# RHnejad/3D_PoseEstimation

Measured on AMD Instinct MI355X. Metric: poses/sec fwd+bwd, 17-joint lifting batch 4096; MPJPE vs ref, higher is better.
Workload: dtype f16x3 (two fp16 planes per fp32 operand, 3 fp16 MFMAs per product, fp32 accumulate); 1 GPU; BASELINE configs[1]: phase1_lifting LinearModel 34-1024-2x(1024-1024)-51, BN+ReLU+Dropout(0.5), one train_1.py step = zero_grad+forward+MSE+backward+AdamW; launch=eager (one call per kernel), per_gpu_batch=4096, global_batch=4096, parallelism=dp1

## Files before the change

3d_poseestimation_amd/_lib.py:

```python
import ctypes
import os

import torch

_HERE = os.path.dirname(os.path.abspath(__file__))
LIB_PATH = os.environ.get("POSELIFT_LIB") or os.path.join(_HERE, "csrc", "libposelift.so")

PL_F32, PL_BF16, PL_BF16X6, PL_F16X3 = 0, 1, 2, 3


GATHER_FN = ctypes.CFUNCTYPE(ctypes.c_int, ctypes.c_void_p, ctypes.c_void_p, ctypes.c_int64, ctypes.c_void_p)


class PLSync(ctypes.Structure):
    _fields_ = [("world", ctypes.c_int32), ("rank", ctypes.c_int32), ("gather", GATHER_FN),
                ("user", ctypes.c_void_p)]


class PLL1Term(ctypes.Structure):
    _fields_ = [("a", ctypes.c_void_p), ("b", ctypes.c_void_p), ("n", ctypes.c_int64),
                ("da", ctypes.c_void_p), ("db", ctypes.c_void_p)]


L1_MAX_TERMS = 8
# ... 84 lines not shown
_D = ctypes.POINTER(PLDesc)
SIGNATURES = {
    "pl_version": (_c.c_int, []),
    "pl_last_error": (_c.c_char_p, []),
    "pl_num_hidden": (_c.c_int64, [_D]),
    "pl_param_tensors": (_c.c_int64, [_D]),
    "pl_param_offset": (_c.c_int64, [_D, _c.c_int64]),
    "pl_param_numel": (_c.c_int64, [_D, _c.c_int64]),
    "pl_param_arena_floats": (_c.c_int64, [_D]),
    "pl_workspace_bytes": (_c.c_size_t, [_D, _c.c_int64]),
    "pl_workspace_view": (_c.c_int, [_D, _c.c_int64, _c.c_int, _c.c_int64,
                                     _c.POINTER(_c.c_size_t), _c.POINTER(_c.c_size_t)]),
    "pl_workspace_bitmap_format": (_c.c_int, [_D, _c.c_int64, _c.c_int64]),
    "pl_lifter_fwd_eval": (_c.c_int, [_D, _P, _P, _c.c_int64, _P, _c.c_size_t, _P]),
    "pl_lifter_fwd_train": (_c.c_int, [_D, _P, _P, _c.c_int64, _P, _c.c_size_t, _c.c_uint64,
                                       _c.c_uint64, _P, _P]),
    "pl_lifter_bwd": (_c.c_int, [_D, _P, _P, _c.c_int64, _P, _c.c_size_t, _P, _P, _P]),
    "pl_lifter_fwd_eval_saved": (_c.c_int, [_D, _P, _P, _c.c_int64, _P, _c.c_size_t, _P]),
    "pl_lifter_bwd_eval": (_c.c_int, [_D, _P, _P, _c.c_int64, _P, _c.c_size_t, _P, _P, _P]),
    "pl_lifter_bwd_layers": (_c.c_int, [_D, _P, _P, _c.c_int64, _P, _c.c_size_t, _P, _P, _c.c_int, _c.c_int, _P]),
    "pl_lifter_train_fwd_bwd": (_c.c_int, [_D, _P, _P, _c.c_int64, _P, _c.c_size_t, _c.c_uint64, _c.c_uint64,
                                           _P, _P, _P, _c.c_int, _c.c_int, _P]),
    "pl_lifter_step_carries_adamw": (_c.c_int, [_D, _c.c_int64]),
    "pl_lifter_train_step": (_c.c_int, [_D, _P, _P, _c.c_int64, _P, _c.c_size_t, _c.c_uint64, _c.c_uint64,
                                        _P, _P, _P, _c.POINTER(PLAdamWStep), _P]),
    "pl_lifter_train_fwd_bwd_crit": (_c.c_int, [_D, _P, _P, _c.c_int64, _P, _c.c_size_t, _c.c_uint64, _c.c_uint64,
                                                _c.POINTER(PLCriterion), _P, _P, _P, _c.c_int, _c.c_int, _P]),
    "pl_lifter_train_step_crit": (_c.c_int, [_D, _P, _P, _c.c_int64, _P, _c.c_size_t, _c.c_uint64, _c.c_uint64,
                                             _c.POINTER(PLCriterion), _P, _P, _P, _c.POINTER(PLAdamWStep), _P]),
    "pl_pose_loss_scratch_bytes": (_c.c_size_t, [_c.c_int64, _c.c_int64, _c.POINTER(PLCriterion)]),
    "pl_pose_loss_fwd_bwd": (_c.c_int, [_P, _P, _c.c_int64, _c.c_int64, _c.POINTER(PLCriterion), _c.c_float, _P, _P, _P, _P]),
    "pl_mse_scratch_bytes": (_c.c_size_t, [_c.c_int64]),
    "pl_mse_fwd_bwd": (_c.c_int, [_P, _P, _c.c_int64, _c.c_float, _P, _P, _P, _P]),
    "pl_l1_scratch_bytes": (_c.c_size_t, [_c.c_int]),
    "pl_l1_terms_fwd_bwd": (_c.c_int, [_c.POINTER(PLL1Term), _c.c_int, _c.c_float, _P, _P, _P]),
    "pl_mpjpe_scratch_bytes": (_c.c_size_t, [_c.c_int64, _c.c_int64]),
    "pl_mpjpe_accum": (_c.c_int, [_P, _P, _c.c_int64, _c.c_int64, _P, _P, _P]),
    "pl_pose_errors": (_c.c_int, [_P, _P, _c.c_int64, _c.c_int64, _P, _P, _P]),
    "pl_pose_errors_host": (_c.c_int, [_P, _P, _c.c_int64, _c.c_int64, _P, _P]),
    "pl_pose_errors_t": (_c.c_int, [_P, _P, _c.c_int64, _c.c_int64, _P, _P, _P, _P, _P]),
    "pl_mpjpe_accum_t": (_c.c_int, [_P, _P, _c.c_int64, _c.c_int64, _P, _P, _P, _P, _P]),
    "pl_pose_metrics_scratch_bytes": (_c.c_size_t, [_c.c_int64, _c.c_int64, _c.c_int, _c.c_int]),
    "pl_pose_metrics_accum": (_c.c_int, [_P, _c.c_int64, _c.c_int64, _P, _c.c_int, _P, _c.c_int, _P, _P, _P, _P, _P]),
    "pl_adamw_flat": (_c.c_int, [_P, _P, _P, _P, _c.c_int64, _c.c_float, _c.c_float, _c.c_float,
                                 _c.c_float, _c.c_float, _c.c_int64, _c.c_float, _P]),
    "pl_adamw_flat_dev": (_c.c_int, [_P, _P, _P, _P, _c.c_int64, _P, _c.c_float, _c.c_float, _c.c_float,
# ... 247 lines not shown
```

3d_poseestimation_amd/csrc/api.hip:

```cpp
#include <stdarg.h>
#include <stdio.h>
#include <stdlib.h>

#include <vector>

#include "adamw.h"
#include "pl_internal.h"

namespace pl {

static thread_local char g_err[512] = "";

void set_error(const char* fmt, ...) {
  va_list ap;
  va_start(ap, fmt);
  vsnprintf(g_err, sizeof(g_err), fmt, ap);
  va_end(ap);
}

namespace {

inline int64_t align_up(int64_t v, int64_t a) { return (v + a - 1) / a * a; }

int check_desc(const PLDesc* d, bool need_arenas) {
// ... 651 lines not shown
namespace pl {
namespace {

struct BwdCtx {
  const PLDesc* d;
  const Ws& w;
  const ParamLayout& P;
  void* ws;
  hipStream_t s;
  const float *x, *dy;
  float *dx, *grads;
  int B, H, O;
  int l_hi, l_lo;
  float kscale;
  bool eval_bn;
  bool small, sl;
  bool top_fused;
  float* loss_out;
  int n_loss_part;
  float loss_inv_n;
  const PLAdamWStep* adam;
  bool adam_rides;
  std::vector<RowJob> jobs;

  float* buf(size_t off) const { return f32(ws, off); }
  float* GA() const { return buf(w.ga); }
  float* GB() const { return buf(w.gb); }
  float* DZ() const { return buf(w.dz); }
  int64_t BH() const { return (int64_t)B * H; }
  const float* gin(int l) const { return (l % 2 == 1) ? GB() : GA(); }
  float* dzbuf(int l) const { return (sl && (l & 1)) ? GB() : DZ(); }
  bool planes_pair(int l) const { return w.layer[l].bwd == Bwd::PlanesPair; }
  float* dzs(int l) const { return (planes_pair(l) && w.pkind == 2) ? buf(w.dzscale) + 2 * l : nullptr; }
  void job(const float* part, float* out, int R, int Hj, int kind, int transK) { jobs.push_back(RowJob{part, out, R, Hj, kind, transK}); }
  SmallBnLayer bn_layer(int l) const {
    const Layer y = layer_of(d, P, grads, l);
    return SmallBnLayer{saved_of(w, ws, l), y.bn.gamma, y.ggamma, y.gbeta, y.gb};
  }
  AdamWRide ride(int64_t lo, int64_t hi) const {
    AdamWRide r = {};
    r.p = const_cast<float*>(d->params) + lo; r.g = grads + lo; r.m = adam->m + lo; r.v = adam->v + lo; r.n = hi - lo;
    r.lr = adam->lr; r.beta1 = adam->beta1; r.beta2 = adam->beta2; r.eps = adam->eps; r.wd = adam->weight_decay; r.gscale = 1.0f;
    r.t = adam->t; r.lr_dev = adam->lr_dev; r.t_dev = adam->t_dev;
    return r;
  }
};

int bnr_amax_pairs(const BwdCtx& c, int l) { return (c.B / 64) * (c.H / (l == c.w.L - 1 ? 32 : 64)); }
BnrEpilogue bnr_of(const BwdCtx& c, int l) {
  const BnSaved sv = saved_of(c.w, c.ws, l);
  const bool scaled = c.w.pkind == 2 && l > 0;
  const BnrSlab slab = bnr_slab(c.d, c.w, c.ws, c.B / 64, scaled ? bnr_amax_pairs(c, l) : 0, c.eval_bn);
  BnrEpilogue b = {};
  b.z = sv.z; b.bits = sv.bits; b.mean = sv.mean; b.rstd = sv.rstd; b.kscale = c.kscale;
  b.part_dy = slab.mine; b.part_dyz = slab.mine + (size_t)(c.B / 64) * c.H;
  b.amax = scaled ? slab.amax_mine : nullptr;
  return b;
}
void set_bnr(GemmArgs& e, const BnrEpilogue& b) {
  e.bnr_z = b.z; e.bnr_bits = b.bits; e.bnr_mean = b.mean; e.bnr_rstd = b.rstd; e.bnr_kscale = b.kscale;
  e.bnr_part_dy = b.part_dy; e.bnr_part_dyz = b.part_dyz; e.bnr_amax = b.amax;
}

int bwd_output(BwdCtx& c) {
  const Ws& w = c.w;
  const int Bi = c.B, H = c.H, O = c.O;
  const float* W2 = c.d->params + c.P.off[4 * w.L];
  float* gW2 = c.grads + c.P.off[4 * w.L];
  float* gb2 = c.grads + c.P.off[4 * w.L + 1];
  const float* h = c.buf(w.act[w.L - 1]);
  if (c.top_fused) {
    SmallTopBwdArgs a = {};
    a.dy = c.dy; a.W2 = W2; a.h = h; a.B = Bi; a.H = H; a.O = O; a.gout = c.GA(); a.dW2 = gW2; a.db2 = gb2;
    a.top = c.bn_layer(w.L - 1); a.kscale = c.kscale; a.dz_top = c.DZ();
    a.mpart = c.buf(w.mse); a.np = c.n_loss_part; a.inv_n = c.loss_inv_n; a.loss = c.loss_out;
    a.tick = const_cast<uint64_t*>(c.d->step_dev);
    return launch_small_top_bwd(a, c.s);
  }
  if (w.out_skinny) {
    SkinnyWideInArgs wi = {};
    wi.X = c.dy; wi.D = h; wi.B = Bi; wi.K = O; wi.H = H; wi.part = c.buf(w.skp_out); wi.xsum = c.buf(w.outpart);
    PL_TRY(launch_skinny_wide_in(wi, c.s));
    c.job(c.buf(w.skp_out), gW2, skinny_in_chunks(Bi), O * H, 0, 0);
    c.job(c.buf(w.outpart), gb2, skinny_in_chunks(Bi), O, 0, 0);
// ... 53 lines not shown
  a.dz = c.planes_pair(l) ? nullptr : c.DZ(); a.part_db = c.buf(w.dbpart[l]);
  a.planes.scale = 1.0f; a.planes.dyn = dzs;
  if (c.planes_pair(l)) { a.planes.h = u16(c.ws, w.dzp); a.planes.l = a.planes.h + c.BH(); a.planes.kind = w.pkind; }
  PL_TRY(launch_bn_bwd_dz(a, c.s));
  c.job(c.buf(w.dbpart[l]), ly.gb, w.RC, H, 0, 0);
  return PL_OK;
}

int bwd_layer_linear(BwdCtx& c, int l) {
  const Ws& w = c.w;
  const PLDesc* d = c.d;
  const int Bi = c.B, H = c.H;
  hipStream_t s = c.s;
  const Layer ly = layer_of(d, c.P, c.grads, l);
  const LayerRoute& r = w.layer[l];
  float* const GA = c.GA();
  float* const GB = c.GB();
  float* const DZ = c.DZ();
  float* const DZl = c.dzbuf(l);
  float* slabs = c.buf(w.slabs);
  const float* a_in = l == 0 ? c.x : (w.planes ? nullptr : c.buf(w.act[l - 1]));
  if (c.planes_pair(l)) {
    float* dzs = c.dzs(l);
    const int64_t BH = c.BH();
    const int splits = tn_splits(H, H, Bi);
    PlanesGemmArgs nn = planes_args(w.pkind, u16(c.ws, w.dzp), BH, H, wplane(d, w, c.ws, l), (int64_t)H * H, H,
                                    (l % 2 == 1) ? GA : GB, Bi, H, H, 1.0f / kWeightPlaneScale, dzs ? dzs + 1 : nullptr);
    if (l % 2 == 1) nn.e.addend = GA;
    if (!c.eval_bn && w.layer[l - 1].bnr_fused) set_bnr(nn.e, bnr_of(c, l - 1));
    float* wsl = c.buf(w.wslab[l]);
    PlanesGemmArgs tn = planes_args(w.pkind, u16(c.ws, w.dzp), BH, H, u16(c.ws, w.actp[l - 1]), BH, H,
                                    splits > 1 ? wsl : ly.gW, H, H, Bi, 1.0f / kActPlaneScale, dzs ? dzs + 1 : nullptr);
    tn.e.split_k = splits;
    PL_TRY(launch_gemm_planes_pair(nn, tn, s));
    if (splits > 1) c.job(wsl, ly.gW, splits, H * H, 1, 0);
  } else if (l > 0) {
    GemmArgs g = {};
    g.A = DZl; g.B = ly.W; g.M = Bi; g.N = H; g.K = H; g.lda = H; g.ldb = H; g.ldc = H; g.split_k = 1;
    if (l % 2 == 1) { g.C = GA; g.addend = GA; } else { g.C = GB; }
    g.arith = arith_of(d);
    g.thin_scratch = slabs; g.thin_scratch_floats = w.slab_floats;
    GemmArgs t = {};
    t.arith = g.arith;
    t.A = DZl; t.B = a_in; t.M = H; t.N = H; t.K = Bi; t.lda = H; t.ldb = H; t.ldc = H; t.split_k = 1; t.C = ly.gW;
    if (c.sl && (r.bwd == Bwd::SmallLayer || r.bwd == Bwd::SmallLayerDw)) {
      const bool dw_rides = r.bwd == Bwd::SmallLayerDw;
      if (l - 1 < c.l_lo) {
        PL_TRY(launch_gemm_f32(kNN, g, s));
        return launch_gemm_f32(kTN, t, s);
      }
      const bool w1 = l == 1 && w.layer[0].bwd == Bwd::InAbove;
      AdamWRide ar = {};
      if (c.adam_rides) ar = c.ride(c.P.off[4 * l + 1], l == w.L - 1 ? c.P.total : c.P.off[4 * (l + 1) + 1]);
      SmallLayerBwdArgs a = {};
      a.dz = DZl; a.W = ly.W; a.B = Bi; a.H = H; a.K = H;
      if (l % 2 == 1) { a.addend = GA; a.gout = GA; }
      a.below = c.bn_layer(l - 1); a.kscale = c.kscale; a.dz_lo = c.dzbuf(l - 1);
      if (dw_rides) { a.a_in = a_in; a.dW = ly.gW; }
// ... 33 lines not shown
                    float* loss_out = nullptr, int n_loss_part = 0, float loss_inv_n = 0.f, const PLAdamWStep* adam = nullptr) {
  PL_TRY(check_desc(d, true));
  if (!x || !dy || !grads) PL_FAIL(PL_EINVAL, "pl_lifter_bwd: null x/dy/flat_grads");
  if (B <= 0) PL_FAIL(PL_ESHAPE, "pl_lifter_bwd: B=%lld", (long long)B);
  const Ws w = plan(d, B);
  PL_TRY(check_ws(w, ws, ws_bytes));
  const ParamLayout P = param_layout(d);
  BwdCtx c = {d, w, P, ws, (hipStream_t)stream, x, dy, dx, grads, (int)B, d->hidden, d->out_dim, l_hi, l_lo};
  c.kscale = eval_bn ? 1.0f : dropout_key(d->p_dropout, 0, 0, 0, nullptr, nullptr).kscale;
  c.eval_bn = eval_bn;
  c.small = !eval_bn && w.bn_small;
  c.sl = !eval_bn && w.small_layer;
  c.top_fused = do_output && !eval_bn && w.top_fused && l_hi == w.L - 1 && l_hi >= l_lo;
  c.loss_out = loss_out;
  c.n_loss_part = n_loss_part;
  c.loss_inv_n = loss_inv_n;
  c.adam = adam;
  c.adam_rides = adam && c.top_fused && l_lo == 0 && w.adam_rides;
  if (do_output) PL_TRY(bwd_output(c));
  for (int l = l_hi; l >= l_lo; --l) {
    PL_TRY(bwd_layer_bn(c, l));
    PL_TRY(bwd_layer_linear(c, l));
  }
  float inv_n = 0.f;
  uint64_t* tick = nullptr;
  if (loss_out && !c.top_fused) {
    c.job(f32(ws, w.mse), loss_out, c.n_loss_part, 1, 2, 0);
    inv_n = loss_inv_n;
    tick = const_cast<uint64_t*>(d->step_dev);
  }
  if (!c.jobs.empty()) PL_TRY(launch_reduce_rows_multi(c.jobs.data(), (int)c.jobs.size(), inv_n, tick, c.s));
  if (adam) {
    const int64_t n = c.adam_rides ? (w.L > 1 ? P.off[4 * 1 + 1] : P.total) : P.total;
    const AdamWArgs a = {const_cast<float*>(d->params), grads, adam->m, adam->v, n,
                         {adam->lr, adam->beta1, adam->beta2, adam->eps, adam->weight_decay, 1.0f, adam->t, adam->lr_dev,
                          adam->t_dev}};
    PL_TRY(launch_adamw(a, c.s));
  }
  return PL_OK;
}

extern "C" int pl_lifter_bwd(const PLDesc* d, const float* x, const float* dy, int64_t B, void* ws,
                             size_t ws_bytes, float* dx, float* grads, void* stream) {
  if (!d) PL_FAIL(PL_EINVAL, "descriptor is NULL");
  return bwd_impl(d, x, dy, B, ws, ws_bytes, dx, grads, stream, true, 2 * d->num_stage, 0);
}
// ... 272 lines not shown
                            double* flops_total) {
  if (!ms_total || !launches || !flops_total) PL_FAIL(PL_EINVAL, "pl_prof_read: null pointer");
  return prof_read(min_flops, max_flops, ms_total, launches, flops_total);
}

static int train_fwd_bwd_impl(const PLDesc* d, const float* x, const float* target, int64_t B, void* ws, size_t ws_bytes,
                              uint64_t seed, uint64_t step, const PLCriterion* crit, float* y, float* loss, float* grads, int hi,
                              int lo, void* stream, const PLAdamWStep* adam);

extern "C" int pl_lifter_train_fwd_bwd_crit(const PLDesc* d, const float* x, const float* target, int64_t B, void* ws,
                                            size_t ws_bytes, uint64_t seed, uint64_t step, const PLCriterion* crit, float* y,
                                            float* loss, float* grads, int hi, int lo, void* stream) {
  return train_fwd_bwd_impl(d, x, target, B, ws, ws_bytes, seed, step, crit, y, loss, grads, hi, lo, stream, nullptr);
}
extern "C" int pl_lifter_train_fwd_bwd(const PLDesc* d, const float* x, const float* target, int64_t B, void* ws,
                                       size_t ws_bytes, uint64_t seed, uint64_t step, float* y, float* loss,
                                       float* grads, int hi, int lo, void* stream) {
  return pl_lifter_train_fwd_bwd_crit(d, x, target, B, ws, ws_bytes, seed, step, nullptr, y, loss, grads, hi, lo, stream);
}

extern "C" int pl_lifter_step_carries_adamw(const PLDesc* d, int64_t B) {
  PL_TRY(check_desc(d, false));
  return B > 0 && plan(d, B).adam_rides ? 1 : 0;
}

extern "C" int pl_lifter_train_step_crit(const PLDesc* d, const float* x, const float* target, int64_t B, void* ws,
                                         size_t ws_bytes, uint64_t seed, uint64_t step, const PLCriterion* crit, float* y,
                                         float* loss, float* grads, const PLAdamWStep* opt, void* stream) {
  if (!opt || !opt->m || !opt->v || (opt->lr_dev != nullptr) != (opt->t_dev != nullptr) || opt->t < (opt->t_dev ? 0 : 1))
    PL_FAIL(PL_EINVAL, "pl_lifter_train_step: bad optimizer description");
  if (!d) PL_FAIL(PL_EINVAL, "descriptor is NULL");
  return train_fwd_bwd_impl(d, x, target, B, ws, ws_bytes, seed, step, crit, y, loss, grads, 1 + 2 * d->num_stage, 0, stream, opt);
}
extern "C" int pl_lifter_train_step(const PLDesc* d, const float* x, const float* target, int64_t B, void* ws, size_t ws_bytes,
                                    uint64_t seed, uint64_t step, float* y, float* loss, float* grads, const PLAdamWStep* opt,
                                    void* stream) {
  return pl_lifter_train_step_crit(d, x, target, B, ws, ws_bytes, seed, step, nullptr, y, loss, grads, opt, stream);
}

static int train_fwd_bwd_impl(const PLDesc* d, const float* x, const float* target, int64_t B, void* ws, size_t ws_bytes,
                              uint64_t seed, uint64_t step, const PLCriterion* crit, float* y, float* loss, float* grads, int hi,
                              int lo, void* stream, const PLAdamWStep* adam) {
  PL_TRY(check_desc(d, true));
  if (!x || !target || !y || !loss || !grads) PL_FAIL(PL_EINVAL, "pl_lifter_train_fwd_bwd: null pointer");
  if (B <= 0) PL_FAIL(PL_ESHAPE, "pl_lifter_train_fwd_bwd: B=%lld", (long long)B);
  PL_TRY(check_range(d, hi, lo, "pl_lifter_train_fwd_bwd"));
// ... 28 lines not shown
```

3d_poseestimation_amd/csrc/gemm_planes.h:

```cpp
#pragma once
#include <hip/hip_runtime.h>
#include <stddef.h>
#include <stdint.h>

#include <type_traits>

namespace plp {

typedef __bf16 bf16x8 __attribute__((ext_vector_type(8)));
typedef _Float16 f16x8 __attribute__((ext_vector_type(8)));
typedef short s16x4 __attribute__((ext_vector_type(4)));
typedef short s16x8 __attribute__((ext_vector_type(8)));

enum PlanesMode { kBf16 = 0, kBf16x6 = 1, kF16x3 = 2 };
template <int MODE> struct ModeCfg;
template <> struct ModeCfg<kBf16>   { static constexpr int NPL = 1, NACC = 1, NPROD = 1; };
template <> struct ModeCfg<kBf16x6> { static constexpr int NPL = 3, NACC = 1, NPROD = 6; };
template <> struct ModeCfg<kF16x3>  { static constexpr int NPL = 2, NACC = 2, NPROD = 3; };
constexpr float kF16LoScale = 2048.0f;

struct PlanesArgs {
  const __bf16* A;
  const __bf16* B;
  float* C;
  int M, N, K;
  int lda, ldb, ldc;
  int split_k;
  size_t a_plane, b_plane;
  int cv_cin, cv_h, cv_w, cv_ho, cv_wo, cv_kw, cv_stride, cv_stride_w, cv_pad_h, cv_pad_w;
};

template <int BKX, int NPL, int NST = 3>
struct PlanesCfg {
  static constexpr int OPP = 128 * BKX * 2;
  static constexpr int STAGE = 2 * NPL * OPP;
  static constexpr int LDS = NST * STAGE;
  static constexpr int NJ = BKX / 16;
  static constexpr int NDMA = 2 * NPL * NJ;
};

#define PLP_BLDS16(rsrc, lp, voff, soff) \
  __builtin_amdgcn_raw_ptr_buffer_load_lds((rsrc), (__attribute__((address_space(3))) void*)(lp), 16, (voff), (soff), 0, 0)

template <int N>
__device__ __forceinline__ void wait_vmcnt() {
  asm volatile("s_waitcnt vmcnt(%0)" ::"n"(N) : "memory");
}

template <int NDS, int NVM, int NMF>
__device__ __forceinline__ void sched_half() {
  constexpr int QV0 = (NDS + 1) / 2;
#pragma unroll
// ... 11 lines not shown
```

3d_poseestimation_amd/csrc/gemm_planes.hip:

```cpp
#include "gemm_planes16.h"
#include "pl_internal.h"
#include "plane_store.h"

namespace pl {
namespace {

struct PlanesKern {
  plp::PlanesArgs p;
  GemmArgs e;
  float out_scale;
  const float* dyn_inv;
  int nt_store;
};

__device__ __forceinline__ float xadd16(const float v) {
  const auto r = __builtin_amdgcn_permlane16_swap(__float_as_uint(v), __float_as_uint(v), false, false);
  return __uint_as_float(r[0]) + __uint_as_float(r[1]);
}
__device__ __forceinline__ float xadd32(const float v) {
  const auto r = __builtin_amdgcn_permlane32_swap(__float_as_uint(v), __float_as_uint(v), false, false);
  return __uint_as_float(r[0]) + __uint_as_float(r[1]);
}
__device__ __forceinline__ float4 xadd_rows(float4 s) {
  s.x = xadd32(xadd16(s.x)); s.y = xadd32(xadd16(s.y)); s.z = xadd32(xadd16(s.z)); s.w = xadd32(xadd16(s.w));
// ... 381 lines not shown
  __device__ __forceinline__ void finish() {
    if constexpr (BNR) {
      const GemmArgs& e = k.e;
      const int N = e.N;
      s1 = xadd_rows(s1);
      s2 = xadd_rows(s2);
      if ((lane >> 4) == 0) {
        *reinterpret_cast<float4*>(e.bnr_part_dy + (size_t)rg * N + col0) = s1;
        *reinterpret_cast<float4*>(e.bnr_part_dyz + (size_t)rg * N + col0) = s2;
      }
      if (e.bnr_amax) {
#pragma unroll
        for (int o = 32; o > 0; o >>= 1) { mxd = fmaxf(mxd, __shfl_xor(mxd, o)); mxz = fmaxf(mxz, __shfl_xor(mxz, o)); }
        if (lane == 0) {
          float* q = e.bnr_amax + ((size_t)rg * (N >> 6) + cb) * 2;
          q[0] = mxd; q[1] = mxz;
        }
      }
    }
  }
};

template <int MODE, bool HAND, bool ADD = false, bool BNR = false>
__global__ __launch_bounds__(512) void planes_gemm_chain_kernel(PlanesKern k0, PlanesKern k1) {
  constexpr int BEHIND = HAND ? plp::kHandBytes : stage_bytes<32>();
  static_assert(ring_bytes<MODE>() + BEHIND <= 160 * 1024 && stage_bytes<32>() <= plp::kHandBytes, "LDS per CU");
  __shared__ __attribute__((aligned(16))) char lds[ring_bytes<MODE>() + BEHIND];
  const int lane = threadIdx.x & 63, wave = threadIdx.x >> 6;
  const int wm = (wave & 3) >> 1, wn = wave & 1;
  float* ldsw = reinterpret_cast<float*>(lds + ring_bytes<MODE>()) + (wave & 3) * 32 * 68;
  auto epi0 = [&](plp::f32x4v (&acc)[plp::ModeCfg<MODE>::NACC][4][4], const int m0, const int n0, const int slice) {
    if constexpr (!HAND) acc_epilogue<MODE, 32, false>(k0, acc, ldsw, m0, n0, slice, wm, wn, lane);
  };
  auto epi1 = [&](plp::f32x4v (&acc)[plp::ModeCfg<MODE>::NACC][4][4], const int m0, const int n0, const int slice) {
    acc_epilogue<MODE, 32, false>(k1, acc, ldsw, m0, n0, slice, wm, wn, lane);
  };
  if constexpr (HAND) {
    ChainHand<MODE, ADD, BNR> hand(k0, reinterpret_cast<float*>(lds + ring_bytes<MODE>()) + (wave & 3) * 64 * 64, lane);
    plp::planes_run16_chain<MODE>(k0.p, k1.p, blockIdx.x, gridDim.x, lds, hand, epi0, epi1);
  } else {
    NoHand hand;
    plp::planes_run16_chain<MODE>(k0.p, k1.p, blockIdx.x, gridDim.x, lds, hand, epi0, epi1);
  }
}

template <int MODE>
__global__ __launch_bounds__(512) void planes_gemm_dual_kernel(PlanesKern k0, PlanesKern k1, int n0) {
  __shared__ __attribute__((aligned(16))) char lds[lds_bytes<MODE>()];
  const int b = blockIdx.x;
  if (b < n0)
    planes_body<false, true, MODE>(k0, b, n0, n0, lds);
  else
    planes_body<true, true, MODE>(k1, b - n0, gridDim.x - n0, gridDim.x - n0, lds);
}

PlanesKern kern_of(const PlanesGemmArgs& a) {
  PlanesKern k = {};
  k.p.A = reinterpret_cast<const __bf16*>(a.A);
  k.p.B = reinterpret_cast<const __bf16*>(a.B);
  k.p.C = a.e.C;
  k.p.M = a.e.M; k.p.N = a.e.N; k.p.K = a.e.K;
  k.p.lda = a.lda; k.p.ldb = a.ldb; k.p.ldc = a.e.ldc;
  k.p.split_k = a.e.split_k;
  k.p.a_plane = (size_t)a.a_plane; k.p.b_plane = (size_t)a.b_plane;
  k.e = a.e;
// ... 68 lines not shown
    }
    if (r.edge) launch(Bool<true>{}, Int<0>{}); else launch(Bool<false>{}, Int<0>{});
  };
  switch (layout) {
    case kNT: one_item(Bool<false>{}, Bool<false>{}, Int<1>{}); break;
    case kNN: one_item(Bool<false>{}, Bool<true>{}, Int<0>{}); break;
    case kTN: one_item(Bool<true>{}, Bool<true>{}, Int<2>{}); break;
    default: PL_FAIL(PL_EINVAL, "gemm_planes: bad layout %d", (int)layout);
  }
  return PL_OK;
}

enum class PairRoute { Chain, ChainHand, Dual };
bool chain_hand_ok(const GemmArgs& e) {
  return e.C && splits_of(e) == 1 && !e.bias && !e.col_scale && !e.relu && !e.resid && !e.cpl_kind && !e.stat_sum && !e.scat_on;
}
PairRoute pair_route(const PlanesGemmArgs& nn, const PlanesGemmArgs& tn) {
  const int ts = splits_of(tn.e);
  const bool chain = grid_of(nn) == grid_of(tn) && nn.e.K % 32 == 0 && nn.e.K >= 64 && tn.e.K % (32 * ts) == 0 && tn.e.K >= 32 * ts;
  if (!chain) return PairRoute::Dual;
  const int nk1 = tn.e.K / (32 * ts);
  return nk1 >= plp::kChainMinNk1 && chain_hand_ok(nn.e) ? PairRoute::ChainHand : PairRoute::Chain;
}
template <int MODE>
void launch_pair(PairRoute r, const PlanesKern& k0, const PlanesKern& k1, int g0, int g1, hipStream_t s) {
  const dim3 block(512);
  if (r == PairRoute::ChainHand) {
    auto launch = [&](auto ADD, auto BNR) {
      hipLaunchKernelGGL((planes_gemm_chain_kernel<MODE, true, decltype(ADD)::value, decltype(BNR)::value>), dim3(g0), block, 0, s, k0, k1);
    };
    auto with_bnr = [&](auto ADD) { if (k0.e.bnr_z) launch(ADD, Bool<true>{}); else launch(ADD, Bool<false>{}); };
    if (k0.e.addend) with_bnr(Bool<true>{}); else with_bnr(Bool<false>{});
  } else if (r == PairRoute::Chain) {
    hipLaunchKernelGGL((planes_gemm_chain_kernel<MODE, false>), dim3(g0), block, 0, s, k0, k1);
  } else {
    hipLaunchKernelGGL((planes_gemm_dual_kernel<MODE>), dim3(g0 + g1), block, 0, s, k0, k1, g0);
  }
}

}

bool planes_gemm_ok(GemmLayout layout, const PlanesGemmArgs& a) {
  const GemmArgs& e = a.e;
  const int splits = splits_of(e);
  if (a.mode != plp::kBf16 && a.mode != plp::kF16x3) return false;
  if (!a.A || !a.B || (!e.C && !e.cpl_kind) || e.M <= 0 || e.N <= 0 || e.K <= 0) return false;
  if (e.cpl_kind && (splits > 1 || !e.cpl_h || (e.cpl_kind == 2 && !e.cpl_l) ||
                     ((reinterpret_cast<uintptr_t>(e.cpl_h) | reinterpret_cast<uintptr_t>(e.cpl_l)) & 7)))
    return false;
  if (e.K % (32 * splits)) return false;
  if (e.conv_cin) {
    if ((layout != kNT && layout != kTN) || e.bnr_z) return false;
    if (e.conv_h <= 0 || e.conv_w <= 0 || e.conv_ho <= 0 || e.conv_wo <= 0 || e.conv_kw <= 0 || e.conv_stride <= 0) return false;
    const int64_t pixels = layout == kNT ? e.M : e.K;
    if (pixels % ((int64_t)e.conv_ho * e.conv_wo)) return false;
    const int64_t xb = pixels / ((int64_t)e.conv_ho * e.conv_wo) * e.conv_h * e.conv_w * e.conv_cin * 2;
    if (xb >= 0x7fffffe0ll) return false;
// ... 40 lines not shown
  } else if (nt && one_slice && e.K % 64 == 0 && e.K >= 1024 && (e.conv_cin == 0 || e.conv_cin % 64 == 0)) {
    r.family = PlanesFamily::Wide;
  } else if (nt && r.nwork >= 2 * ncu) {
    r.family = PlanesFamily::Persistent;
  } else {
    r.family = PlanesFamily::OneItem;
  }
  r.persist = r.family != PlanesFamily::OneItem && r.nwork >= 2 * ncu;
  r.grid = r.persist ? ncu : r.nwork;
  return r;
}

int launch_gemm_planes(GemmLayout layout, const PlanesGemmArgs& a, hipStream_t s) {
  if (!planes_gemm_ok(layout, a)) PL_FAIL(PL_ESHAPE, "gemm_planes: unsupported problem %dx%dx%d (layout %d, mode %d)", a.e.M, a.e.N, a.e.K, (int)layout, a.mode);
  const PlanesKern k = kern_of(a);
  const PlanesRoute r = planes_route(layout, a, cu_count());
  void* prof = prof_begin_flops(2.0 * a.e.M * a.e.N * a.e.K, s);
  PL_TRY(a.mode == plp::kF16x3 ? launch_routed<plp::kF16x3>(layout, r, k, s) : launch_routed<plp::kBf16>(layout, r, k, s));
  prof_end(prof, s);
  PL_CHECK_LAUNCH("gemm_planes");
  return PL_OK;
}

int launch_gemm_planes_pair(const PlanesGemmArgs& nn, const PlanesGemmArgs& tn, hipStream_t s) {
  if (!planes_gemm_ok(kNN, nn) || !planes_gemm_ok(kTN, tn) || nn.mode != tn.mode || is_edge(nn) || is_edge(tn))
    PL_FAIL(PL_ESHAPE, "gemm_planes_pair: unsupported problems");
  const PlanesKern k0 = kern_of(nn), k1 = kern_of(tn);
  const PairRoute r = pair_route(nn, tn);
  void* prof = prof_begin_flops(2.0 * nn.e.M * nn.e.N * nn.e.K + 2.0 * tn.e.M * tn.e.N * tn.e.K, s);
  if (nn.mode == plp::kF16x3) launch_pair<plp::kF16x3>(r, k0, k1, grid_of(nn), grid_of(tn), s);
  else launch_pair<plp::kBf16>(r, k0, k1, grid_of(nn), grid_of(tn), s);
  prof_end(prof, s);
  PL_CHECK_LAUNCH(r == PairRoute::Dual ? "gemm_planes_dual" : "gemm_planes_chain");
  return PL_OK;
}

}
```

3d_poseestimation_amd/csrc/gemm_planes16.h:

```cpp
#pragma once
#include <utility>

#include "gemm_planes.h"

namespace plp {

typedef float f32x4v __attribute__((ext_vector_type(4)));

__device__ __forceinline__ int kc16_swz(int row) { return (0 - (row >> 2)) & 3; }

template <bool KS>
__device__ __forceinline__ uint32_t glds_lane_off16(int rb, int lane, int ld, int left = 0x7fffffff) {
  if (!KS) {
    const int row = rb * 16 + (lane >> 2);
    const int ch = (lane & 3) ^ kc16_swz(row);
    return (uint32_t)(min(row, left - 1) * ld * 2 + ch * 16);
  }
  const int krow = rb * 4 + (lane >> 4);
  const int ch = (lane & 15) ^ ((((lane >> 4) & 3) << 2) | (rb & 3));
  return (uint32_t)(krow * ld * 2 + min(ch, (left >> 3) - 1) * 16);
}

template <bool KS>
struct FragAddr16 {
// ... 336 lines not shown
        if (kt + 1 < nk) step(kt + 1, P1{}, F_{});
      }
    }
    epi(acc, m0, n0, slice);
  }
#undef PLP16_READ_A
#undef PLP16_READ_B
#undef PLP16_MFS
#undef PLP16_ROWS
}

constexpr int kChainChunks = 16;
constexpr int kChainAhead = 3;
constexpr int kChainFirst = 0;
constexpr int kChainMinNk1 = kChainFirst + kChainChunks + kChainAhead + 1;
static_assert(kChainFirst + kChainAhead >= 3, "the hand-off block is complete after the barrier of item-1 iteration 2");
constexpr int kHandBytes = 4 * 64 * 64 * 4;

__device__ __forceinline__ int hand_idx(const int row, const int col) { return row * 64 + (col ^ (((row >> 2) & 3) << 4)); }

template <class F, int... J>
__device__ __forceinline__ void unroll_ints(F&& f, std::integer_sequence<int, J...>) { (f(std::integral_constant<int, J>{}), ...); }

template <int MODE, class Hand, class Epi0, class Epi1>
__device__ __forceinline__ void planes_run16_chain(const PlanesArgs& p0, const PlanesArgs& p1, const int block_id, const int nwork,
                                                   char* __restrict__ lds, Hand& hand, Epi0&& epi0, Epi1&& epi1) {
  static_assert(MODE == kF16x3 || MODE == kBf16, "two fp16 planes or one bf16 plane");
  constexpr int NPL = ModeCfg<MODE>::NPL, NACC = ModeCfg<MODE>::NACC;
  using Cf = PlanesCfg<32, NPL, 3>;
  const int tid = threadIdx.x;
  const int lane = tid & 63;
  const int wave = __builtin_amdgcn_readfirstlane(tid >> 6);
  const bool loader = wave >= 4;
  const int lw = wave & 3;
  const int wm = (wave & 3) >> 1, wn = wave & 1;
  int w = block_id;
  if ((nwork & 7) == 0) w = (block_id & 7) * (nwork >> 3) + (block_id >> 3);
  const int tn0 = p0.N / 128;
  const int m00 = (w / tn0) * 128, n00 = (w % tn0) * 128;
  const int nk0 = p0.K / 32;
  const int tn1 = p1.N / 128;
  const int splits = p1.split_k > 1 ? p1.split_k : 1;
  const int ntiles1 = nwork / splits;
  const int slice = w / ntiles1, t1 = w - slice * ntiles1;
  const int m01 = (t1 / tn1) * 128, n01 = (t1 % tn1) * 128;
  const int per = ((p1.K / 32 + splits - 1) / splits) * 32;
  const int kbeg1 = min(slice * per, p1.K);
  const int nk1 = (min(kbeg1 + per, p1.K) - kbeg1) / 32;
  const int total = nk0 + nk1;
// ... 36 lines not shown
#pragma unroll
        for (int j = 0; j < 2; ++j) {
          PLP_BLDS16(ra0[pl], d + pl * Cf::OPP + j * 4096, oa0[j], sa);
          PLP_BLDS16(rb0[pl], d + (NPL + pl) * Cf::OPP + j * 4096, ob0[j], sb);
        }
      sw = next_stage(sw);
    };
    auto issue1 = [&](const int kt) {
      char* d = lds + sw + lw * 1024;
      const int sa = kt * ga1, sb = kt * gb1;
#pragma unroll
      for (int pl = 0; pl < NPL; ++pl)
#pragma unroll
        for (int j = 0; j < 2; ++j) {
          PLP_BLDS16(ra1[pl], d + pl * Cf::OPP + j * 4096, oa1[j], sa);
          PLP_BLDS16(rb1[pl], d + (NPL + pl) * Cf::OPP + j * 4096, ob1[j], sb);
        }
      sw = next_stage(sw);
    };
    issue0(0);
    issue0(1);
    wait_vmcnt<Cf::NDMA>();
    barrier();
    for (int g = 0; g + 2 < nk0; ++g) { issue0(g + 2); wait_vmcnt<Cf::NDMA>(); barrier(); }
    if constexpr (!Hand::kOn) {
      for (int kt = 0; kt < nk1; ++kt) { issue1(kt); wait_vmcnt<Cf::NDMA>(); barrier(); }
    } else {
      hand.begin(m00, n00, wm, wn);
      for (int kt = 0; kt < kChainFirst; ++kt) { issue1(kt); wait_vmcnt<Cf::NDMA>(); barrier(); }
      unroll_ints([&](auto jc) {
        constexpr int J = decltype(jc)::value;
        issue1(kChainFirst + J);
        __builtin_amdgcn_sched_barrier(0);
        hand.chunk(jc);
        wait_vmcnt<Hand::vm_ops(J - 1) + Cf::NDMA + Hand::vm_ops(J)>();
        barrier();
      }, std::make_integer_sequence<int, kChainChunks + kChainAhead>{});
      for (int kt = kChainFirst + kChainChunks + kChainAhead; kt < nk1; ++kt) { issue1(kt); wait_vmcnt<Cf::NDMA>(); barrier(); }
    }
    wait_vmcnt<0>(); barrier();
    wait_vmcnt<0>(); barrier();
    if constexpr (Hand::kOn) hand.finish();
    return;
  }

  FragAddr16<false> fa_kc;
  FragAddr16<true> fa_ks;
// ... 413 lines not shown
```

3d_poseestimation_amd/csrc/pl_internal.h:

```cpp
#pragma once
#include <hip/hip_runtime.h>
#include <stddef.h>
#include <stdint.h>

#include <type_traits>

#include "../../include/poselift.h"
#include "adamw.h"
#include "philox.h"
#include "pose_criterion.h"

namespace pl {

constexpr int kWave = 64;
__device__ __forceinline__ bool relu_on(float v) { return !(v <= 0.f); }
__device__ __forceinline__ float relu_f(float v) { return __builtin_elementwise_maximum(v, 0.f); }
__device__ __forceinline__ float max_nan(float a, float b) { return __builtin_elementwise_maximum(a, b); }
template <bool V> using Bool = std::integral_constant<bool, V>;
template <int V> using Int = std::integral_constant<int, V>;

void set_error(const char* fmt, ...);

#define PL_FAIL(code, ...)        \
  do {                            \
// ... 83 lines not shown
constexpr float kConvActPlaneScale = 1.0f / 64.0f;

struct PlanesGemmArgs {
  GemmArgs e;
  const unsigned short* A;
  const unsigned short* B;
  int64_t a_plane, b_plane;
  int lda, ldb;
  int mode;
  float out_scale;
  const float* dyn_inv;
};
bool planes_gemm_ok(GemmLayout layout, const PlanesGemmArgs& a);
enum class PlanesFamily { OneItem, Persistent, Wide, T64 };
struct PlanesRoute {
  PlanesFamily family;
  bool persist;
  bool edge;
  int conv;
  int grid, nwork;
};
PlanesRoute planes_route(GemmLayout layout, const PlanesGemmArgs& a, int ncu);
int launch_gemm_planes(GemmLayout layout, const PlanesGemmArgs& a, hipStream_t s);
int launch_gemm_planes_pair(const PlanesGemmArgs& nn, const PlanesGemmArgs& tn, hipStream_t s);
int launch_split_planes(const float* x, int64_t n, const PlaneOut& out, hipStream_t s);
int plane_out_of(int mode, void* planes, int64_t n, float scale, const float* dyn, PlaneOut* po, const char* who);

int launch_gemm_f32(GemmLayout layout, const GemmArgs& a, hipStream_t s);
constexpr int kThinGemmMaxM = 512;
bool thin_gemm_ok(GemmLayout layout, const GemmArgs& a);
size_t thin_gemm_scratch_floats(int M, int N, int K);
int launch_gemm_thin(GemmLayout layout, const GemmArgs& a, hipStream_t s);
int launch_gemm_f32_pair(const GemmArgs& nn, const GemmArgs& tn, hipStream_t s);
int gemm_stat_groups(int M);
int prof_enable(int on);
void* prof_begin_flops(double flops, hipStream_t s);
void prof_end(void* rec, hipStream_t s);
int prof_read(double min_flops, double max_flops, double* ms_total, int64_t* launches, double* flops_total);

inline int bitmap_words_per_row(int H) { return ((H + 255) / 256) * 4; }

struct BnParams {
  const float *gamma, *beta;
  float eps, momentum;
  float *running_mean, *running_var;
  int64_t* batches;
};
// ... 251 lines not shown
```

include/poselift.h:

```cpp
#ifndef POSELIFT_H_
#define POSELIFT_H_

#include <stddef.h>
#include <stdint.h>

#ifdef __cplusplus
extern "C" {
#endif

#define PL_VERSION 118

typedef enum PLStatus {
  PL_OK = 0,
  PL_EINVAL = -1,
  PL_ESHAPE = -2,
  PL_EDTYPE = -3,
  PL_EBATCH = -4,
  PL_EHIP = -5,
  PL_EWORKSPACE = -6,
  PL_ESYNC = -7
} PLStatus;

typedef enum PLDtype { PL_F32 = 0, PL_BF16 = 1, PL_BF16X6 = 2, PL_F16X3 = 3 } PLDtype;

typedef int (*PLGatherFn)(void* user, float* buf, int64_t floats_per_rank, void* stream);
typedef struct PLSync {
  int32_t world;
  int32_t rank;
  PLGatherFn gather;
  void* user;
} PLSync;

typedef struct PLDesc {
// ... 45 lines not shown
int pl_lifter_fwd_eval_saved(const PLDesc* d, const float* x, float* y, int64_t B,
                             void* workspace, size_t workspace_bytes, void* stream);
int pl_lifter_bwd_eval(const PLDesc* d, const float* x, const float* dy, int64_t B,
                       void* workspace, size_t workspace_bytes, float* dx, float* flat_grads, void* stream);

int pl_lifter_bwd_layers(const PLDesc* d, const float* x, const float* dy, int64_t B,
                         void* workspace, size_t workspace_bytes, float* dx,
                         float* flat_grads, int hi, int lo, void* stream);

int pl_lifter_train_fwd_bwd(const PLDesc* d, const float* x, const float* target, int64_t B,
                            void* workspace, size_t workspace_bytes, uint64_t seed, uint64_t step,
                            float* y, float* loss, float* flat_grads, int hi, int lo, void* stream);

typedef struct PLAdamWStep {
  float* m;
  float* v;
  float lr;
  const float* lr_dev;
  float beta1, beta2, eps, weight_decay;
  int64_t t;
  const uint64_t* t_dev;
} PLAdamWStep;
int pl_lifter_step_carries_adamw(const PLDesc* d, int64_t B);
int pl_lifter_train_step(const PLDesc* d, const float* x, const float* target, int64_t B, void* workspace,
                         size_t workspace_bytes, uint64_t seed, uint64_t step, float* y, float* loss, float* flat_grads,
                         const PLAdamWStep* opt, void* stream);

typedef enum PLCriterionKind { PL_CRIT_MSE = 0, PL_CRIT_L1 = 1, PL_CRIT_SMOOTH_L1 = 2, PL_CRIT_MPJPE = 3 } PLCriterionKind;
typedef struct PLCriterion {
  int32_t kind;
  int32_t group;
  float beta;
  const float* weights;
} PLCriterion;
size_t pl_pose_loss_scratch_bytes(int64_t B, int64_t O, const PLCriterion* crit);
int pl_pose_loss_fwd_bwd(const float* pred, const float* tgt, int64_t B, int64_t O, const PLCriterion* crit, float grad_scale,
                         float* dpred , float* loss, void* scratch, void* stream);
int pl_lifter_train_fwd_bwd_crit(const PLDesc* d, const float* x, const float* target, int64_t B, void* workspace,
                                 size_t workspace_bytes, uint64_t seed, uint64_t step, const PLCriterion* crit, float* y,
                                 float* loss, float* flat_grads, int hi, int lo, void* stream);
int pl_lifter_train_step_crit(const PLDesc* d, const float* x, const float* target, int64_t B, void* workspace,
                              size_t workspace_bytes, uint64_t seed, uint64_t step, const PLCriterion* crit, float* y,
                              float* loss, float* flat_grads, const PLAdamWStep* opt, void* stream);

int pl_softargmax3d_nhwc_fwd(const float* logits, int64_t B, int64_t J, int64_t H, int64_t W,
                             float* coords, float* stats, void* stream);
// ... 384 lines not shown
```

Baseline: 7.059 million poses/s.

## Carry split-K weight-gradient slab sum inside next layer's backward GEMM pair

Layer l's split-K dW partial slabs were summed by a separate row-reduction job. They are now deferred and reduced inside the next lower layer's chained NN/TN planes GEMM kernel. The reduction's loads and stores are interleaved into the first-GEMM prologue loop, between DMA issues, with vmcnt waits adjusted to match. This hides the reduction's memory traffic under the GEMM and removes a separate pass, at the cost of extra registers and stricter shape and alignment conditions in the hand-tuned chain kernel.

After: 7.223 million poses/s, median of 6. +2.3%, better.

```diff
diff --git a/3d_poseestimation_amd/_lib.py b/3d_poseestimation_amd/_lib.py
--- a/3d_poseestimation_amd/_lib.py
+++ b/3d_poseestimation_amd/_lib.py
@@ -130,6 +130,7 @@
     "pl_lifter_train_fwd_bwd": (_c.c_int, [_D, _P, _P, _c.c_int64, _P, _c.c_size_t, _c.c_uint64, _c.c_uint64,
                                            _P, _P, _P, _c.c_int, _c.c_int, _P]),
     "pl_lifter_step_carries_adamw": (_c.c_int, [_D, _c.c_int64]),
+    "pl_lifter_bwd_slab_rides": (_c.c_int, [_D, _c.c_int64, _c.c_int, _c.c_int]),
     "pl_lifter_train_step": (_c.c_int, [_D, _P, _P, _c.c_int64, _P, _c.c_size_t, _c.c_uint64, _c.c_uint64,
                                         _P, _P, _P, _c.POINTER(PLAdamWStep), _P]),
     "pl_lifter_train_fwd_bwd_crit": (_c.c_int, [_D, _P, _P, _c.c_int64, _P, _c.c_size_t, _c.c_uint64, _c.c_uint64,
diff --git a/3d_poseestimation_amd/csrc/api.hip b/3d_poseestimation_amd/csrc/api.hip
--- a/3d_poseestimation_amd/csrc/api.hip
+++ b/3d_poseestimation_amd/csrc/api.hip
@@ -697,6 +697,7 @@
   const PLAdamWStep* adam;
   bool adam_rides;
   std::vector<RowJob> jobs;
+  RowJob pending = {};
 
   float* buf(size_t off) const { return f32(ws, off); }
   float* GA() const { return buf(w.ga); }
@@ -735,6 +736,23 @@
 void set_bnr(GemmArgs& e, const BnrEpilogue& b) {
   e.bnr_z = b.z; e.bnr_bits = b.bits; e.bnr_mean = b.mean; e.bnr_rstd = b.rstd; e.bnr_kscale = b.kscale;
   e.bnr_part_dy = b.part_dy; e.bnr_part_dyz = b.part_dyz; e.bnr_amax = b.amax;
+}
+
+void pair_problems(const Ws& w, int H, int B, float* g_out, float* dw_out, PlanesGemmArgs& nn, PlanesGemmArgs& tn) {
+  const int64_t BH = (int64_t)B * H;
+  nn = planes_args(w.pkind, nullptr, BH, H, nullptr, (int64_t)H * H, H, g_out, B, H, H, 1.0f / kWeightPlaneScale, nullptr);
+  tn = planes_args(w.pkind, nullptr, BH, H, nullptr, BH, H, dw_out, H, H, B, 1.0f / kActPlaneScale, nullptr);
+  tn.e.split_k = tn_splits(H, H, B);
+}
+bool slab_sum_rides_below(const Ws& w, int H, int B, int l, int l_lo) {
+  if (l - 1 < l_lo || l - 1 < 1 || l >= w.L) return false;
+  if (w.layer[l].bwd != Bwd::PlanesPair || w.layer[l - 1].bwd != Bwd::PlanesPair) return false;
+  const int splits = tn_splits(H, H, B);
+  if (splits <= 1) return false;
+  static float placeholder[4];
+  PlanesGemmArgs nn, tn;
+  pair_problems(w, H, B, placeholder, placeholder, nn, tn);
+  return planes_pair_carries_slab_sum(nn, tn, splits, (int64_t)H * H);
 }
 
 int bwd_output(BwdCtx& c) {
@@ -834,18 +852,23 @@
   const float* a_in = l == 0 ? c.x : (w.planes ? nullptr : c.buf(w.act[l - 1]));
   if (c.planes_pair(l)) {
     float* dzs = c.dzs(l);
-    const int64_t BH = c.BH();
     const int splits = tn_splits(H, H, Bi);
-    PlanesGemmArgs nn = planes_args(w.pkind, u16(c.ws, w.dzp), BH, H, wplane(d, w, c.ws, l), (int64_t)H * H, H,
-                                    (l % 2 == 1) ? GA : GB, Bi, H, H, 1.0f / kWeightPlaneScale, dzs ? dzs + 1 : nullptr);
+    float* wsl = c.buf(w.wslab[l]);
+    PlanesGemmArgs nn, tn;
+    pair_problems(w, H, Bi, (l % 2 == 1) ? GA : GB, splits > 1 ? wsl : ly.gW, nn, tn);
+    nn.A = tn.A = u16(c.ws, w.dzp);
+    nn.B = wplane(d, w, c.ws, l);
+    tn.B = u16(c.ws, w.actp[l - 1]);
+    if (w.pkind == 2) nn.dyn_inv = tn.dyn_inv = dzs ? dzs + 1 : nullptr;
     if (l % 2 == 1) nn.e.addend = GA;
     if (!c.eval_bn && w.layer[l - 1].bnr_fused) set_bnr(nn.e, bnr_of(c, l - 1));
-    float* wsl = c.buf(w.wslab[l]);
-    PlanesGemmArgs tn = planes_args(w.pkind, u16(c.ws, w.dzp), BH, H, u16(c.ws, w.actp[l - 1]), BH, H,
-                                    splits > 1 ? wsl : ly.gW, H, H, Bi, 1.0f / kActPlaneScale, dzs ? dzs + 1 : nullptr);
-    tn.e.split_k = splits;
-    PL_TRY(launch_gemm_planes_pair(nn, tn, s));
-    if (splits > 1) c.job(wsl, ly.gW, splits, H * H, 1, 0);
+    const SlabSum above = {c.pending.part, c.pending.out, c.pending.R, (int64_t)c.pending.H};
+    PL_TRY(launch_gemm_planes_pair(nn, tn, c.pending.R > 0 ? &above : nullptr, s));
+    c.pending = RowJob{};
+    if (splits > 1) {
+      const RowJob sum = {wsl, ly.gW, splits, H * H, 1, 0};
+      if (slab_sum_rides_below(w, H, Bi, l, c.l_lo)) c.pending = sum; else c.jobs.push_back(sum);
+    }
   } else if (l > 0) {
     GemmArgs g = {};
     g.A = DZl; g.B = ly.W; g.M = Bi; g.N = H; g.K = H; g.lda = H; g.ldb = H; g.ldc = H; g.split_k = 1;
@@ -925,6 +948,7 @@
     PL_TRY(bwd_layer_bn(c, l));
     PL_TRY(bwd_layer_linear(c, l));
   }
+  if (c.pending.R > 0) c.jobs.push_back(c.pending);
   float inv_n = 0.f;
   uint64_t* tick = nullptr;
   if (loss_out && !c.top_fused) {
@@ -1243,6 +1267,16 @@
 extern "C" int pl_lifter_step_carries_adamw(const PLDesc* d, int64_t B) {
   PL_TRY(check_desc(d, false));
   return B > 0 && plan(d, B).adam_rides ? 1 : 0;
+}
+
+extern "C" int pl_lifter_bwd_slab_rides(const PLDesc* d, int64_t B, int hi, int lo) {
+  PL_TRY(check_desc(d, false));
+  PL_TRY(check_range(d, hi, lo, "pl_lifter_bwd_slab_rides"));
+  if (B <= 0 || B > INT32_MAX) return 0;
+  const Ws w = plan(d, B);
+  int n = 0;
+  for (int l = hi < w.L ? hi : w.L - 1; l > lo; --l) n += pl::slab_sum_rides_below(w, d->hidden, (int)B, l, lo) ? 1 : 0;
+  return n;
 }
 
 extern "C" int pl_lifter_train_step_crit(const PLDesc* d, const float* x, const float* target, int64_t B, void* ws,
diff --git a/3d_poseestimation_amd/csrc/gemm_planes.h b/3d_poseestimation_amd/csrc/gemm_planes.h
--- a/3d_poseestimation_amd/csrc/gemm_planes.h
+++ b/3d_poseestimation_amd/csrc/gemm_planes.h
@@ -28,6 +28,13 @@
   int split_k;
   size_t a_plane, b_plane;
   int cv_cin, cv_h, cv_w, cv_ho, cv_wo, cv_kw, cv_stride, cv_stride_w, cv_pad_h, cv_pad_w;
+};
+
+struct SlabRide {
+  const float* part;
+  float* out;
+  long long stride;
+  int R, n4;
 };
 
 template <int BKX, int NPL, int NST = 3>
diff --git a/3d_poseestimation_amd/csrc/gemm_planes.hip b/3d_poseestimation_amd/csrc/gemm_planes.hip
--- a/3d_poseestimation_amd/csrc/gemm_planes.hip
+++ b/3d_poseestimation_amd/csrc/gemm_planes.hip
@@ -427,7 +427,7 @@
 };
 
 template <int MODE, bool HAND, bool ADD = false, bool BNR = false>
-__global__ __launch_bounds__(512) void planes_gemm_chain_kernel(PlanesKern k0, PlanesKern k1) {
+__global__ __launch_bounds__(512) void planes_gemm_chain_kernel(PlanesKern k0, PlanesKern k1, plp::SlabRide ride) {
   constexpr int BEHIND = HAND ? plp::kHandBytes : stage_bytes<32>();
   static_assert(ring_bytes<MODE>() + BEHIND <= 160 * 1024 && stage_bytes<32>() <= plp::kHandBytes, "LDS per CU");
   __shared__ __attribute__((aligned(16))) char lds[ring_bytes<MODE>() + BEHIND];
@@ -442,10 +442,10 @@
   };
   if constexpr (HAND) {
     ChainHand<MODE, ADD, BNR> hand(k0, reinterpret_cast<float*>(lds + ring_bytes<MODE>()) + (wave & 3) * 64 * 64, lane);
-    plp::planes_run16_chain<MODE>(k0.p, k1.p, blockIdx.x, gridDim.x, lds, hand, epi0, epi1);
+    plp::planes_run16_chain<MODE>(k0.p, k1.p, ride, blockIdx.x, gridDim.x, lds, hand, epi0, epi1);
   } else {
     NoHand hand;
-    plp::planes_run16_chain<MODE>(k0.p, k1.p, blockIdx.x, gridDim.x, lds, hand, epi0, epi1);
+    plp::planes_run16_chain<MODE>(k0.p, k1.p, ride, blockIdx.x, gridDim.x, lds, hand, epi0, epi1);
   }
 }
 
@@ -560,17 +560,23 @@
   const int nk1 = tn.e.K / (32 * ts);
   return nk1 >= plp::kChainMinNk1 && chain_hand_ok(nn.e) ? PairRoute::ChainHand : PairRoute::Chain;
 }
+bool pair_carries_slab_sum(const PlanesGemmArgs& nn, const PlanesGemmArgs& tn, int slabs, int64_t n) {
+  if (pair_route(nn, tn) != PairRoute::ChainHand) return false;
+  const int nk0 = nn.e.K / 32;
+  return slabs == plp::kRideSlabs && n == (int64_t)plp::kRideChunks * 4 * 64 * 4 * grid_of(nn) && nk0 >= plp::kRideMinNk0;
+}
 template <int MODE>
-void launch_pair(PairRoute r, const PlanesKern& k0, const PlanesKern& k1, int g0, int g1, hipStream_t s) {
+void launch_pair(PairRoute r, const PlanesKern& k0, const PlanesKern& k1, const plp::SlabRide& ride, int g0, int g1, hipStream_t s) {
   const dim3 block(512);
   if (r == PairRoute::ChainHand) {
     auto launch = [&](auto ADD, auto BNR) {
-      hipLaunchKernelGGL((planes_gemm_chain_kernel<MODE, true, decltype(ADD)::value, decltype(BNR)::value>), dim3(g0), block, 0, s, k0, k1);
+      hipLaunchKernelGGL((planes_gemm_chain_kernel<MODE, true, decltype(ADD)::value, decltype(BNR)::value>), dim3(g0), block, 0, s, k0, k1,
+                         ride);
     };
     auto with_bnr = [&](auto ADD) { if (k0.e.bnr_z) launch(ADD, Bool<true>{}); else launch(ADD, Bool<false>{}); };
     if (k0.e.addend) with_bnr(Bool<true>{}); else with_bnr(Bool<false>{});
   } else if (r == PairRoute::Chain) {
-    hipLaunchKernelGGL((planes_gemm_chain_kernel<MODE, false>), dim3(g0), block, 0, s, k0, k1);
+    hipLaunchKernelGGL((planes_gemm_chain_kernel<MODE, false>), dim3(g0), block, 0, s, k0, k1, plp::SlabRide{});
   } else {
     hipLaunchKernelGGL((planes_gemm_dual_kernel<MODE>), dim3(g0 + g1), block, 0, s, k0, k1, g0);
   }
@@ -657,14 +663,26 @@
   return PL_OK;
 }
 
-int launch_gemm_planes_pair(const PlanesGemmArgs& nn, const PlanesGemmArgs& tn, hipStream_t s) {
+bool planes_pair_carries_slab_sum(const PlanesGemmArgs& nn, const PlanesGemmArgs& tn, int slabs, int64_t n) {
+  return pair_carries_slab_sum(nn, tn, slabs, n);
+}
+
+int launch_gemm_planes_pair(const PlanesGemmArgs& nn, const PlanesGemmArgs& tn, const SlabSum* sum, hipStream_t s) {
   if (!planes_gemm_ok(kNN, nn) || !planes_gemm_ok(kTN, tn) || nn.mode != tn.mode || is_edge(nn) || is_edge(tn))
     PL_FAIL(PL_ESHAPE, "gemm_planes_pair: unsupported problems");
   const PlanesKern k0 = kern_of(nn), k1 = kern_of(tn);
   const PairRoute r = pair_route(nn, tn);
+  plp::SlabRide ride = {};
+  if (sum) {
+    if (!sum->part || !sum->out || !pair_carries_slab_sum(nn, tn, sum->slabs, sum->n))
+      PL_FAIL(PL_ESHAPE, "gemm_planes_pair: cannot carry a sum of %d slabs of %lld floats", sum->slabs, (long long)sum->n);
+    if ((reinterpret_cast<uintptr_t>(sum->part) | reinterpret_cast<uintptr_t>(sum->out)) & 15)
+      PL_FAIL(PL_EINVAL, "gemm_planes_pair: slab sum alignment");
+    ride.part = sum->part; ride.out = sum->out; ride.stride = sum->n; ride.R = sum->slabs; ride.n4 = (int)(sum->n / 4);
+  }
   void* prof = prof_begin_flops(2.0 * nn.e.M * nn.e.N * nn.e.K + 2.0 * tn.e.M * tn.e.N * tn.e.K, s);
-  if (nn.mode == plp::kF16x3) launch_pair<plp::kF16x3>(r, k0, k1, grid_of(nn), grid_of(tn), s);
-  else launch_pair<plp::kBf16>(r, k0, k1, grid_of(nn), grid_of(tn), s);
+  if (nn.mode == plp::kF16x3) launch_pair<plp::kF16x3>(r, k0, k1, ride, grid_of(nn), grid_of(tn), s);
+  else launch_pair<plp::kBf16>(r, k0, k1, ride, grid_of(nn), grid_of(tn), s);
   prof_end(prof, s);
   PL_CHECK_LAUNCH(r == PairRoute::Dual ? "gemm_planes_dual" : "gemm_planes_chain");
   return PL_OK;
diff --git a/3d_poseestimation_amd/csrc/gemm_planes16.h b/3d_poseestimation_amd/csrc/gemm_planes16.h
--- a/3d_poseestimation_amd/csrc/gemm_planes16.h
+++ b/3d_poseestimation_amd/csrc/gemm_planes16.h
@@ -382,9 +382,58 @@
 template <class F, int... J>
 __device__ __forceinline__ void unroll_ints(F&& f, std::integer_sequence<int, J...>) { (f(std::integral_constant<int, J>{}), ...); }
 
+constexpr int kRideSlabs = 4;
+constexpr int kRideChunks = 4;
+constexpr int kRideFirst = 12;
+constexpr int kRideMinNk0 = kRideFirst + kRideChunks + kChainAhead + 2;
+
+struct SlabRider {
+  static constexpr int D = kChainAhead;
+  static constexpr int vm_ops(int j) { return (j >= 0 && j < kRideChunks ? kRideSlabs : 0) + (j >= D && j - D < kRideChunks ? 1 : 0); }
+  const float* src;
+  float* dst;
+  size_t stride, step;
+  float4 a[D], b1[D], b2[D], b3[D];
+
+  __device__ __forceinline__ void begin(const SlabRide& r, const int wv, const int nwaves, const int lane) {
+    const size_t o = ((size_t)wv * 64 + lane) * 4;
+    src = r.part + o;
+    dst = r.out + o;
+    stride = (size_t)r.stride;
+    step = (size_t)nwaves * 64 * 4;
+  }
+
+  template <int J>
+  __device__ __forceinline__ void chunk(std::integral_constant<int, J>) {
+    auto ld = [](const float* p) {
+      const f32x4v t = __builtin_nontemporal_load(reinterpret_cast<const f32x4v*>(p));
+      return make_float4(t[0], t[1], t[2], t[3]);
+    };
+    float4 na, n1, n2, n3;
+    if constexpr (J < kRideChunks) {
+      const float* q = src + J * step;
+      na = ld(q);
+      n1 = ld(q + stride);
+      n2 = ld(q + 2 * stride);
+      n3 = ld(q + 3 * stride);
+    }
+    if constexpr (J >= D && J - D < kRideChunks) {
+      constexpr int it = J - D, sl = it % D;
+      float4 v = a[sl];
+      v.x += b1[sl].x; v.y += b1[sl].y; v.z += b1[sl].z; v.w += b1[sl].w;
+      v.x += b2[sl].x; v.y += b2[sl].y; v.z += b2[sl].z; v.w += b2[sl].w;
+      v.x += b3[sl].x; v.y += b3[sl].y; v.z += b3[sl].z; v.w += b3[sl].w;
+      asm volatile("" : "+v"(v.x), "+v"(v.y), "+v"(v.z), "+v"(v.w));
+      const f32x4v t = {v.x, v.y, v.z, v.w};
+      __builtin_nontemporal_store(t, reinterpret_cast<f32x4v*>(dst + it * step));
+    }
+    if constexpr (J < kRideChunks) { a[J % D] = na; b1[J % D] = n1; b2[J % D] = n2; b3[J % D] = n3; }
+  }
+};
+
 template <int MODE, class Hand, class Epi0, class Epi1>
-__device__ __forceinline__ void planes_run16_chain(const PlanesArgs& p0, const PlanesArgs& p1, const int block_id, const int nwork,
-                                                   char* __restrict__ lds, Hand& hand, Epi0&& epi0, Epi1&& epi1) {
+__device__ __forceinline__ void planes_run16_chain(const PlanesArgs& p0, const PlanesArgs& p1, const SlabRide& ride, const int block_id,
+                                                   const int nwork, char* __restrict__ lds, Hand& hand, Epi0&& epi0, Epi1&& epi1) {
   static_assert(MODE == kF16x3 || MODE == kBf16, "two fp16 planes or one bf16 plane");
   constexpr int NPL = ModeCfg<MODE>::NPL, NACC = ModeCfg<MODE>::NACC;
   using Cf = PlanesCfg<32, NPL, 3>;
@@ -467,7 +516,24 @@
     issue0(1);
     wait_vmcnt<Cf::NDMA>();
     barrier();
-    for (int g = 0; g + 2 < nk0; ++g) { issue0(g + 2); wait_vmcnt<Cf::NDMA>(); barrier(); }
+    bool rides = false;
+    if constexpr (Hand::kOn) rides = ride.part != nullptr;
+    if (!rides) {
+      for (int g = 0; g + 2 < nk0; ++g) { issue0(g + 2); wait_vmcnt<Cf::NDMA>(); barrier(); }
+    } else {
+      SlabRider rd;
+      rd.begin(ride, block_id * 4 + lw, nwork * 4, lane);
+      for (int g = 0; g < kRideFirst; ++g) { issue0(g + 2); wait_vmcnt<Cf::NDMA>(); barrier(); }
+      unroll_ints([&](auto jc) {
+        constexpr int J = decltype(jc)::value;
+        issue0(kRideFirst + J + 2);
+        __builtin_amdgcn_sched_barrier(0);
+        rd.chunk(jc);
+        wait_vmcnt<SlabRider::vm_ops(J - 1) + Cf::NDMA + SlabRider::vm_ops(J)>();
+        barrier();
+      }, std::make_integer_sequence<int, kRideChunks + kChainAhead>{});
+      for (int g = kRideFirst + kRideChunks + kChainAhead; g + 2 < nk0; ++g) { issue0(g + 2); wait_vmcnt<Cf::NDMA>(); barrier(); }
+    }
     if constexpr (!Hand::kOn) {
       for (int kt = 0; kt < nk1; ++kt) { issue1(kt); wait_vmcnt<Cf::NDMA>(); barrier(); }
     } else {
diff --git a/3d_poseestimation_amd/csrc/pl_internal.h b/3d_poseestimation_amd/csrc/pl_internal.h
--- a/3d_poseestimation_amd/csrc/pl_internal.h
+++ b/3d_poseestimation_amd/csrc/pl_internal.h
@@ -129,7 +129,9 @@
 };
 PlanesRoute planes_route(GemmLayout layout, const PlanesGemmArgs& a, int ncu);
 int launch_gemm_planes(GemmLayout layout, const PlanesGemmArgs& a, hipStream_t s);
-int launch_gemm_planes_pair(const PlanesGemmArgs& nn, const PlanesGemmArgs& tn, hipStream_t s);
+struct SlabSum { const float* part; float* out; int slabs; int64_t n; };
+bool planes_pair_carries_slab_sum(const PlanesGemmArgs& nn, const PlanesGemmArgs& tn, int slabs, int64_t n);
+int launch_gemm_planes_pair(const PlanesGemmArgs& nn, const PlanesGemmArgs& tn, const SlabSum* sum, hipStream_t s);
 int launch_split_planes(const float* x, int64_t n, const PlaneOut& out, hipStream_t s);
 int plane_out_of(int mode, void* planes, int64_t n, float scale, const float* dyn, PlaneOut* po, const char* who);
 
diff --git a/include/poselift.h b/include/poselift.h
--- a/include/poselift.h
+++ b/include/poselift.h
@@ -8,7 +8,7 @@
 extern "C" {
 #endif
 
-#define PL_VERSION 118
+#define PL_VERSION 119
 
 typedef enum PLStatus {
   PL_OK = 0,
@@ -100,6 +100,7 @@
   const uint64_t* t_dev;
 } PLAdamWStep;
 int pl_lifter_step_carries_adamw(const PLDesc* d, int64_t B);
+int pl_lifter_bwd_slab_rides(const PLDesc* d, int64_t B, int hi, int lo);
 int pl_lifter_train_step(const PLDesc* d, const float* x, const float* target, int64_t B, void* workspace,
                          size_t workspace_bytes, uint64_t seed, uint64_t step, float* y, float* loss, float* flat_grads,
                          const PLAdamWStep* opt, void* stream);
```
